# tub-rip/cmax_slam

Measured on AMD Instinct MI355X. Metric: warped-events/sec/GPU (1M ev, 640x480 IWE) + CMax iters/sec, higher is better.
Workload: dtype f64

## Files before the change

### cmax_slam_amd/csrc/cmx_binning.hip

```cpp
#include <mutex>
#include <cstring>

#include <rocprim/rocprim.hpp>

#include "cmx_internal.hpp"
#include "cmx_warp.hpp"
#include "cmx_fixed.hpp"
#include "cmx_tilepass.hpp"
#include "cmx_fusedgather.hpp"
#include "cmx_selfserve.hpp"

namespace cmx {

__device__ __forceinline__ uint32_t tile_key(int xx, int yy, bool ok, int W, int H, int tiles_x, uint32_t sentinel) {
  if (!ok) {
    if (xx < 1 - kBinMargin || xx >= W - 2 + kBinMargin || yy < 1 - kBinMargin || yy >= H - 2 + kBinMargin) return sentinel;
    xx = min(max(xx, 1), W - 3);
    yy = min(max(yy, 1), H - 3);
  }
  return (uint32_t)((yy / kBinTile) * tiles_x + xx / kBinTile);
}

__global__ __launch_bounds__(256) void fe_bin_keys_kernel(FeSplatArgs a, int tiles_x, int ntiles, uint32_t *keys,
                                                          uint32_t *idx) {
  fe_resolve_omega(a);
  for (int i = blockIdx.x * 256 + threadIdx.x; i < a.n; i += gridDim.x * 256) {
    const FeWarp w = fe_warp_event<false>(a, i);
    keys[i] = tile_key(w.xx, w.yy, w.ok, a.W, a.H, tiles_x, (uint32_t)ntiles);
    idx[i] = (uint32_t)i;
  }
}
__global__ __launch_bounds__(256) void be_bin_keys_kernel(BeSplatArgs a, int tiles_x, int ntiles, uint32_t *keys,
                                                          uint32_t *idx) {
  for (int i = blockIdx.x * 256 + threadIdx.x; i < a.n; i += gridDim.x * 256) {
    const BeWarp w = be_warp_event<0>(a, i);
    const uint32_t t = tile_key(w.xx, w.yy, w.ok, a.Wp, a.Hp, tiles_x, (uint32_t)ntiles);
    keys[i] = t == (uint32_t)ntiles ? (uint32_t)(2 * ntiles) : 2 * t + (w.is_old ? 0u : 1u);
    idx[i] = (uint32_t)i;
  }
}
static int grid_for(int n) {
  int b = (n + 255) / 256;
  return b < 1 ? 1 : (b > 2048 ? 2048 : b);
}
void launch_fe_bin_keys(const FeSplatArgs &a, int tiles_x, int ntiles, uint32_t *keys, uint32_t *idx, hipStream_t s) {
  hipLaunchKernelGGL(fe_bin_keys_kernel, dim3(grid_for(a.n)), dim3(256), 0, s, a, tiles_x, ntiles, keys, idx);
}
void launch_be_bin_keys(const BeSplatArgs &a, int tiles_x, int ntiles, uint32_t *keys, uint32_t *idx, hipStream_t s) {
  hipLaunchKernelGGL(be_bin_keys_kernel, dim3(grid_for(a.n)), dim3(256), 0, s, a, tiles_x, ntiles, keys, idx);
}

int sort_pairs_u32(void *temp, size_t *temp_bytes, const uint32_t *kin, uint32_t *kout, const uint32_t *vin,
                   uint32_t *vout, unsigned n, int end_bit, hipStream_t s) {
  return (int)rocprim::radix_sort_pairs(temp, *temp_bytes, kin, kout, vin, vout, n, 0, end_bit, s);
}

__global__ __launch_bounds__(256) void apply_perm_kernel(const uint32_t *xy, const uint32_t *idx_sorted, int per_batch,
                                                         int n, uint32_t *sxy, uint32_t *sbatch) {
  for (int j = blockIdx.x * 256 + threadIdx.x; j < n; j += gridDim.x * 256) {
    const uint32_t i = idx_sorted[j];
    sxy[j] = xy[i];
    sbatch[j] = i / (uint32_t)per_batch;
  }
}
void launch_apply_perm(const uint32_t *xy, const uint32_t *idx_sorted, int per_batch, int n, uint32_t *sxy,
                       uint32_t *sbatch, hipStream_t s) {
  hipLaunchKernelGGL(apply_perm_kernel, dim3(grid_for(n)), dim3(256), 0, s, xy, idx_sorted, per_batch, n, sxy, sbatch);
}

__global__ void tile_lower_bound_kernel(const uint32_t *keys, int n, int count, int *tile_start) {
  const int t = blockIdx.x * blockDim.x + threadIdx.x;
  if (t >= count) return;
  int lo = 0, hi = n;
  while (lo < hi) {
    const int mid = (lo + hi) >> 1;
    if (keys[mid] < (uint32_t)t) lo = mid + 1;
    else hi = mid;
  }
  tile_start[t] = lo;
}
void launch_tile_lower_bound(const uint32_t *keys_sorted, int n, int count, int *tile_start, hipStream_t s) {
  hipLaunchKernelGGL(tile_lower_bound_kernel, dim3((count + 255) / 256), dim3(256), 0, s, keys_sorted, n, count, tile_start);
}

constexpr int kCountSortMaxBins = 16400;
constexpr int kBinBlock = 1024;
constexpr int kBinMaxSlices = 512;
extern __shared__ int hist_sh[];

__device__ __forceinline__ void hist_zero(int nbins) {
  for (int k = threadIdx.x; k < nbins; k += kBinBlock) hist_sh[k] = 0;
  __syncthreads();
}
__device__ __forceinline__ void hist_store_row(int nbins, int *table) {
  __syncthreads();
  int *row = table + (size_t)blockIdx.x * nbins;
  for (int k = threadIdx.x; k < nbins; k += kBinBlock) row[k] = hist_sh[k];
}
__global__ __launch_bounds__(kBinBlock) void fe_bin_hist_kernel(FeSplatArgs a, int tiles_x, int ntiles, int per_block,
                                                                uint32_t *keys, int *table) {
  fe_resolve_omega(a);
  hist_zero(ntiles + 1);
  const int beg = blockIdx.x * per_block, end = min(a.n, beg + per_block);
  for (int i = beg + threadIdx.x; i < end; i += kBinBlock) {
    const FeWarp w = fe_warp_event<false>(a, i);
    const uint32_t key = tile_key(w.xx, w.yy, w.ok, a.W, a.H, tiles_x, (uint32_t)ntiles);
    keys[i] = key;
    atomicAdd(&hist_sh[key], 1);
  }
  hist_store_row(ntiles + 1, table);
}
__global__ __launch_bounds__(kBinBlock) void be_bin_hist_kernel(BeSplatArgs a, int tiles_x, int ntiles, int per_block,
                                                                uint32_t *keys, int *table) {
  hist_zero(2 * ntiles + 1);
  const int beg = blockIdx.x * per_block, end = min(a.n, beg + per_block);
  for (int i = beg + threadIdx.x; i < end; i += kBinBlock) {
    const BeWarp w = be_warp_event<0>(a, i);
    const uint32_t t = tile_key(w.xx, w.yy, w.ok, a.Wp, a.Hp, tiles_x, (uint32_t)ntiles);
    const uint32_t key = t == (uint32_t)ntiles ? (uint32_t)(2 * ntiles) : 2 * t + (w.is_old ? 0u : 1u);
    keys[i] = key;
    atomicAdd(&hist_sh[key], 1);
  }
  hist_store_row(2 * ntiles + 1, table);
}
__global__ __launch_bounds__(256) void column_scan_kernel(int *table, int nbins, int nslices, int *total) {
  const int k = blockIdx.x * 256 + threadIdx.x;
  if (k >= nbins) return;
  int run = 0, s = 0;
  for (; s + 8 <= nslices; s += 8) {
    int v[8];
#pragma unroll
    for (int q = 0; q < 8; q++) v[q] = table[(size_t)(s + q) * nbins + k];
#pragma unroll
    for (int q = 0; q < 8; q++) {
      table[(size_t)(s + q) * nbins + k] = run;
      run += v[q];
    }
  }
  for (; s < nslices; s++) {
    const int v = table[(size_t)s * nbins + k];
    table[(size_t)s * nbins + k] = run;
    run += v;
  }
  total[k] = run;
}
__global__ __launch_bounds__(kBinBlock) void scan_bins_kernel(const int *total, int nbins, int *tile_start) {
  __shared__ int wave_tot[kBinBlock / 64];
  const int tid = threadIdx.x, lane = tid & 63, wave = tid >> 6;
  const int per = (nbins + kBinBlock - 1) / kBinBlock;
  const int k0 = min(nbins, tid * per), k1 = min(nbins, k0 + per);
  int sum = 0;
  for (int k = k0; k < k1; k++) sum += total[k];
  int incl = sum;
#pragma unroll
  for (int o = 1; o < 64; o <<= 1) {
    const int v = __shfl_up(incl, o, 64);
    if (lane >= o) incl += v;
  }
// ... 160 lines not shown
    __shared__ int nact_sh;
    if (tid == 0) nact_sh = 0;
    int *nch = ts_sh;
    int mine[(kRankSortMax + 1023) / 1024];
#pragma unroll
    for (int q = 0; q < (kRankSortMax + 1023) / 1024; q++) {
      const int t = tid + q * 1024;
      int len = t < ntiles ? tile_start[t + 1] - tile_start[t] : 0;
      if (len < 0) len = 0;
      mine[q] = len / M + (len % M ? 1 : 0);
    }
    __syncthreads();
#pragma unroll
    for (int q = 0; q < (kRankSortMax + 1023) / 1024; q++)
      if (tid + q * 1024 < ntiles) nch[tid + q * 1024] = mine[q];
    __syncthreads();
    for (int t = tid; t < ntiles; t += 1024) {
      const int tx = t % tiles_x, ty = t / tiles_x;
      int sum = 0;
      for (int dy = -kFuseNbr; dy <= kFuseNbr; dy++)
        for (int dx = -kFuseNbr; dx <= kFuseNbr; dx++) {
          const int ux = tx + dx, uy = ty + dy;
          if (ux >= 0 && ux < tiles_x && uy >= 0 && uy < fused.tiles_y) sum += nch[uy * tiles_x + ux];
        }
      for (int h = 0; h < kFuseStrips; h++) {
        const int u = t * kFuseStrips + h;
        fused.nbr_expected[u] = sum;
        fused.nbr_cnt[(size_t)u * kFuseCntStride] = 0u;
        fused.partials[u] = 0.0;
        fused.partials[ntiles * kFuseStrips + u] = 0.0;
      }
      if (sum > 0) atomicAdd(&nact_sh, kFuseStrips);
    }
    __syncthreads();
    if (tid == 0) {
      if (fused.n_active) *fused.n_active = nact_sh;
      if (fused.tiles_done) *fused.tiles_done = 0u;
    }
  }
}
bool fused_tables_ok(int ntiles, int planes_per_tile) { return planes_per_tile == 1 && ntiles + 2 <= kRankSortMax + 2; }
void launch_build_chunks(const int *tile_start, int ntiles, int planes_per_tile, int tiles_x, int margin, int M, Chunk *chunks,
                         int *count, unsigned long long *count_host, unsigned binning_id, hipStream_t s, const FusedTables *fused) {
  FusedTables ft{};
  if (fused && fused_tables_ok(ntiles, planes_per_tile)) ft = *fused;
  hipLaunchKernelGGL(build_chunks_kernel, dim3(1), dim3(1024), 0, s, tile_start, ntiles, planes_per_tile, tiles_x, margin, M,
                     chunks, count, count_host, binning_id, ft);
}

__device__ __forceinline__ void lds_add_fix(fix_t *p, fix_t v) {
  __hip_atomic_fetch_add(p, v, __ATOMIC_RELAXED, __HIP_MEMORY_SCOPE_WORKGROUP);
}
__device__ __forceinline__ void vote4_lds(fix_t *win, int lx, int ly, float dx, float dy) {
  fix_t *q = win + ly * kBinStride + lx;
  lds_add_fix(q, to_fix((1.f - dx) * (1.f - dy)));
  lds_add_fix(q + 1, to_fix(dx * (1.f - dy)));
  lds_add_fix(q + kBinStride, to_fix((1.f - dx) * dy));
  lds_add_fix(q + kBinStride + 1, to_fix(dx * dy));
}

__global__ __launch_bounds__(256) void fixed_to_float_kernel(fix_t *fixed, float *planes, size_t n) {
  for (size_t i = (size_t)blockIdx.x * 256 + threadIdx.x; i < n; i += (size_t)gridDim.x * 256) {
    const fix_t v = fixed[i];
    if (v != 0ull) {
      planes[i] = (float)((double)v * kFixInv);
      fixed[i] = 0ull;
    }
  }
}
void launch_fixed_to_float(unsigned long long *fixed, float *planes, size_t n, hipStream_t s) {
  if (n == 0) return;
  size_t blocks = (n + 1023) / 1024;
  if (blocks > 4096) blocks = 4096;
  hipLaunchKernelGGL(fixed_to_float_kernel, dim3((unsigned)blocks), dim3(256), 0, s, fixed, planes, n);
}

static_assert(kBinWindow * kBinWindow % 256 == 0, "window cells per thread");
constexpr int kUnroll = 2;

#ifndef CMX_FE_SPLAT_NT
#define CMX_FE_SPLAT_NT 512
#endif
constexpr int kFeSplatNT = CMX_FE_SPLAT_NT;
static_assert(kBinWindow * kBinWindow % kFeSplatNT == 0, "window cells per thread");
static_assert(sizeof(fix_t) * kBinWindow * kBinStride >= kTpLdsBytes, "the fused tile pass reuses the vote window's LDS");
constexpr unsigned long long kFuseTimeoutTicks = 200000ull;
template <bool FIXED, bool STREAM, int FUSE>
__device__ __forceinline__ void fe_splat_lds_body(FeSplatArgs &a, const BinnedEvents &b, const FusedArgs &f) {
  __shared__ __attribute__((aligned(16))) fix_t win[kBinWindow * kBinStride];
  if (wg_stop_requested(a.skip)) return;
  if (FUSE == 2 && (int)blockIdx.x >= b.nchunks + f.tiles_x * f.tiles_y * kFuseStrips) {
    __shared__ FgSmem fg_sm;
    fused_gather_role<kFeSplatNT>(a, b, f, (int)blockIdx.x - b.nchunks - f.tiles_x * f.tiles_y * kFuseStrips, fg_sm);
    return;
  }
  if ((FUSE == 1 || FUSE == 2) && (int)blockIdx.x >= b.nchunks) {
    const int t = (int)blockIdx.x - b.nchunks;
    const unsigned expected = (unsigned)f.nbr_expected[t];
    if (f.trace && threadIdx.x == 0) { f.trace[8 * (size_t)blockIdx.x] = wall_clock64(); f.trace[8 * (size_t)blockIdx.x + 3] = expected ? 2 : 3; }
    if (expected == 0u || (f.debug & 1)) return;
    __shared__ int ok_sh;
    auto wait_inputs = [&]() -> bool {
      if (threadIdx.x == 0) {
        const unsigned long long t0 = wall_clock64();
        int ok = 1;
        while (__hip_atomic_load(f.nbr_cnt + (size_t)t * kFuseCntStride, __ATOMIC_RELAXED, __HIP_MEMORY_SCOPE_AGENT) < expected) {
          if (f.debug & 8) __builtin_amdgcn_s_sleep(32); else if (f.debug & 16) __builtin_amdgcn_s_sleep(127); else __builtin_amdgcn_s_sleep(2);
          if (wall_clock64() - t0 > kFuseTimeoutTicks) { ok = 0; break; }
        }
        if (ok) __hip_atomic_store(f.nbr_cnt + (size_t)t * kFuseCntStride, 0u, __ATOMIC_RELAXED, __HIP_MEMORY_SCOPE_AGENT);
        else atomicOr(b.fallback, kFuseIncomplete);
// ... 12 lines not shown
        __hip_atomic_store(f.tile_done + (size_t)t * kFuseCntStride, f.seq, __ATOMIC_RELAXED, __HIP_MEMORY_SCOPE_AGENT);
        __hip_atomic_fetch_add(f.tiles_done, 1u, __ATOMIC_RELAXED, __HIP_MEMORY_SCOPE_AGENT);
      }
    }
    if (f.trace && threadIdx.x == 0) { asm volatile("s_waitcnt vmcnt(0)" ::: "memory"); f.trace[8 * (size_t)blockIdx.x + 2] = wall_clock64(); }
    return;
  }
  fe_resolve_omega(a);
  Chunk c = b.chunks[blockIdx.x];
  if (FUSE && f.trace && threadIdx.x == 0) { f.trace[8 * (size_t)blockIdx.x] = wall_clock64(); f.trace[8 * (size_t)blockIdx.x + 3] = 0; }
  const bool has_chunk = (int)blockIdx.x < *b.nchunks_dev;
  if (!has_chunk) {
    if (FUSE != 3) return;
    c = Chunk{-200000000, -200000000, 0, 0, 0, -1};
  }
  const bool has_win = c.wx0 > -100000000;
  const int tid = threadIdx.x;
  __shared__ unsigned sfall;
  if (tid == 0) sfall = 0;
  if (has_win)
    for (int p = tid; p < kBinWindow * kBinStride; p += kFeSplatNT) win[p] = 0ull;
  __syncthreads();
  unsigned nfall = 0;
  for (int j0 = c.beg + tid; j0 < c.end; j0 += kFeSplatNT * kUnroll) {
    bool act[kUnroll];
    double px[kUnroll], py[kUnroll], pz[kUnroll], dt[kUnroll];
    if (STREAM) {
#pragma unroll
      for (int u = 0; u < kUnroll; u++) {
        const int j = j0 + u * kFeSplatNT;
        act[u] = j < c.end;
        const int jj = act[u] ? j : c.beg;
        const double2 v = *reinterpret_cast<const double2 *>(b.sb + 2 * (size_t)jj);
        px[u] = v.x; py[u] = v.y; pz[u] = 1.0;
        dt[u] = b.sdt[jj];
      }
    } else {
      uint32_t e[kUnroll], bi[kUnroll];
#pragma unroll
      for (int u = 0; u < kUnroll; u++) {
        const int j = j0 + u * kFeSplatNT;
        act[u] = j < c.end;
        e[u] = act[u] ? b.sxy[j] : 0u;
        bi[u] = act[u] ? b.sbatch[j] : 0u;
      }
#pragma unroll
      for (int u = 0; u < kUnroll; u++) {
        load_bearing(a, (int)(e[u] & 0xffff), (int)((e[u] >> 16) & 0x7fff), px[u], py[u], pz[u]);
        dt[u] = a.batch_dt[bi[u]];
      }
    }
#pragma unroll
    for (int u = 0; u < kUnroll; u++) {
      const FeWarp w = fe_warp_math<false>(a, px[u], py[u], pz[u], dt[u]);
      if (act[u] && w.ok) {
        const int lx = w.xx - c.wx0, ly = w.yy - c.wy0;
        if (has_win && lx >= 0 && lx < kBinWindow - 1 && ly >= 0 && ly < kBinWindow - 1) {
          vote4_lds(win, lx, ly, w.dx, w.dy);
        } else {
          if (FIXED) vote4_global_fix(b.fixed, a.W, w.xx, w.yy, w.dx, w.dy);
          else vote4_global(a.planes, a.W, w.xx, w.yy, w.dx, w.dy);
          nfall++;
          if (!has_win || lx < kBinMargin - kFuseReach || lx + 1 > kBinMargin + kBinTile - 1 + kFuseReach || ly < kBinMargin - kFuseReach ||
              ly + 1 > kBinMargin + kBinTile - 1 + kFuseReach)
            nfall |= kFuseUnsafe;
        }
      }
    }
  }
  if (nfall) {
    atomicAdd(&sfall, nfall & kFuseCountMask);
    if (nfall & kFuseUnsafe) atomicOr(&sfall, kFuseUnsafe);
  }
  __syncthreads();
  if (tid == 0 && sfall) {
    if (sfall & kFuseCountMask) atomicAdd(b.fallback, sfall & kFuseCountMask);
    if (sfall & kFuseUnsafe) atomicOr(b.fallback, kFuseUnsafe);
  }
  if (has_win) {
    constexpr int kCells = kBinWindow * kBinWindow / kFeSplatNT;
    fix_t cell[kCells];
#pragma unroll
    for (int k = 0; k < kCells; k++) {
      const int p = tid + kFeSplatNT * k, ly = p / kBinWindow, lx = p - ly * kBinWindow;
      cell[k] = win[ly * kBinStride + lx];
    }
#pragma unroll
    for (int k = 0; k < kCells; k++) {
      const fix_t v = cell[k];
      if (v != 0ull) {
        const int p = tid + kFeSplatNT * k, ly = p / kBinWindow, lx = p - ly * kBinWindow;
        const size_t at = (size_t)(c.wy0 + ly) * a.W + (c.wx0 + lx);
        if (FIXED) atomicAdd(b.fixed + at, v);
        else atomic_add_f32(a.planes + at, (float)((double)v * kFixInv));
      }
    }
  }
  if (FUSE) {
    asm volatile("s_waitcnt vmcnt(0)" ::: "memory");
    __syncthreads();
    constexpr int kSide = 2 * kFuseNbr + 1;
    if (c.tile >= 0 && tid < kSide * kSide * kFuseStrips && !(f.debug & 4)) {
      const int q = tid / kFuseStrips, h = tid % kFuseStrips;
      const int tx = c.tile % f.tiles_x + (q % kSide - kFuseNbr), ty = c.tile / f.tiles_x + (q / kSide - kFuseNbr);
      if (tx >= 0 && tx < f.tiles_x && ty >= 0 && ty < f.tiles_y)
        __hip_atomic_fetch_add(f.nbr_cnt + (size_t)((ty * f.tiles_x + tx) * kFuseStrips + h) * kFuseCntStride, 1u, __ATOMIC_RELAXED,
                               __HIP_MEMORY_SCOPE_AGENT);
    }
    if (f.trace && tid == 0) { f.trace[8 * (size_t)blockIdx.x + 1] = wall_clock64(); f.trace[8 * (size_t)blockIdx.x + 3] = 1; }
  }
// ... 60 lines not shown
  } else {
    if (stream) launch_fe_splat_lds_t<false, true, 0>(a, b, none, s, t0, t1);
    else launch_fe_splat_lds_t<false, false, 0>(a, b, none, s, t0, t1);
  }
}

template <bool FIXED>
__global__ __launch_bounds__(256) void be_splat_lds_kernel(BeSplatArgs a, BinnedEvents b) {
  __shared__ fix_t win[kBinWindow * kBinStride];
  const Chunk c = b.chunks[blockIdx.x];
  if ((int)blockIdx.x >= *b.nchunks_dev) return;
  const bool has_win = c.wx0 > -100000000;
  const int tid = threadIdx.x;
  const size_t np = (size_t)a.Wp * a.Hp;
  __shared__ unsigned sfall;
  if (tid == 0) sfall = 0;
  if (has_win)
    for (int p = tid; p < kBinWindow * kBinStride; p += 256) win[p] = 0ull;
  __syncthreads();
  unsigned nfall = 0;
  constexpr int U = 2;
  for (int j0 = c.beg + tid; j0 < c.end; j0 += 256 * U) {
    uint32_t e[U], bi[U];
    bool act[U];
#pragma unroll
    for (int u = 0; u < U; u++) {
      const int j = j0 + u * 256;
      act[u] = j < c.end;
      e[u] = act[u] ? b.sxy[j] : 0u;
      bi[u] = act[u] ? b.sbatch[j] : 0u;
    }
    double rx[U], ry[U], rz[U];
#pragma unroll
    for (int u = 0; u < U; u++) {
      double R[9];
      const double *Rp = a.poseR[bi[u]].R;
#pragma unroll
      for (int k = 0; k < 9; k++) R[k] = Rp[k];
      if (b.sb) {
        const int jj = act[u] ? j0 + u * 256 : c.beg;
        const double2 v = *reinterpret_cast<const double2 *>(b.sb + 2 * (size_t)jj);
        be_rotate<true>(R, v.x, v.y, 1.0, rx[u], ry[u], rz[u]);
      } else {
        double b0, b1, b2;
        load_bearing(a, (int)(e[u] & 0xffff), (int)((e[u] >> 16) & 0x7fff), b0, b1, b2);
        be_rotate<false>(R, b0, b1, b2, rx[u], ry[u], rz[u]);
      }
    }
#pragma unroll
    for (int u = 0; u < U; u++) {
      const BeWarp w = be_project<0>(a, e[u], (int)bi[u], rx[u], ry[u], rz[u]);
      if (act[u] && w.ok) {
        const int lx = w.xx - c.wx0, ly = w.yy - c.wy0;
        if (has_win && lx >= 0 && lx < kBinWindow - 1 && ly >= 0 && ly < kBinWindow - 1) {
          vote4_lds(win, lx, ly, w.dx, w.dy);
        } else {
          if (FIXED) vote4_global_fix(b.fixed + (w.is_old ? 0 : np), a.Wp, w.xx, w.yy, w.dx, w.dy);
          else vote4_global(a.planes + (w.is_old ? 0 : np), a.Wp, w.xx, w.yy, w.dx, w.dy);
          if (b.tflags) {
            b.tflags[(w.yy / kTileY) * b.tflags_tiles_x + w.xx / kTileX] = 1;
            b.tflags[(w.yy / kTileY) * b.tflags_tiles_x + (w.xx + 1) / kTileX] = 1;
            b.tflags[((w.yy + 1) / kTileY) * b.tflags_tiles_x + w.xx / kTileX] = 1;
            b.tflags[((w.yy + 1) / kTileY) * b.tflags_tiles_x + (w.xx + 1) / kTileX] = 1;
          }
          nfall++;
        }
      }
    }
  }
  if (nfall) atomicAdd(&sfall, nfall);
  __syncthreads();
  if (tid == 0 && sfall) atomicAdd(b.fallback, sfall);
  if (has_win) {
    const size_t plane_off = c.plane ? np : 0;
    constexpr int kCells = kBinWindow * kBinWindow / 256;
    fix_t cell[kCells];
#pragma unroll
    for (int k = 0; k < kCells; k++) {
      const int p = tid + 256 * k, ly = p / kBinWindow, lx = p - ly * kBinWindow;
      cell[k] = win[ly * kBinStride + lx];
    }
#pragma unroll
    for (int k = 0; k < kCells; k++) {
      const fix_t v = cell[k];
      if (v != 0ull) {
        const int p = tid + 256 * k, ly = p / kBinWindow, lx = p - ly * kBinWindow;
        const size_t at = plane_off + (size_t)(c.wy0 + ly) * a.Wp + (c.wx0 + lx);
        if (FIXED) atomicAdd(b.fixed + at, v);
        else atomic_add_f32(a.planes + at, (float)((double)v * kFixInv));
        if (b.tflags) b.tflags[((c.wy0 + ly) / kTileY) * b.tflags_tiles_x + (c.wx0 + lx) / kTileX] = 1;
      }
    }
  }
}
void launch_be_splat_lds(const BeSplatArgs &a, const BinnedEvents &b, hipStream_t s, hipEvent_t t0, hipEvent_t t1) {
  if (b.nchunks <= 0) return;
  if (b.fixed) {
    if (t0 || t1) hipExtLaunchKernelGGL(be_splat_lds_kernel<true>, dim3(b.nchunks), dim3(256), 0, s, t0, t1, 0, a, b);
    else hipLaunchKernelGGL(be_splat_lds_kernel<true>, dim3(b.nchunks), dim3(256), 0, s, a, b);
  } else {
    if (t0 || t1) hipExtLaunchKernelGGL(be_splat_lds_kernel<false>, dim3(b.nchunks), dim3(256), 0, s, t0, t1, 0, a, b);
    else hipLaunchKernelGGL(be_splat_lds_kernel<false>, dim3(b.nchunks), dim3(256), 0, s, a, b);
  }
}

}
```

### cmax_slam_amd/csrc/cmx_kernels.hip

```cpp
#include "../../include/cmax_hip.h"
#include "cmx_internal.hpp"
#include "cmx_warp.hpp"

#define CMX_LAUNCH(kernel, grid, block, lds, stream, t0, t1, ...)                                            \
  do {                                                                                                      \
    if ((t0) || (t1)) hipExtLaunchKernelGGL(kernel, grid, block, lds, stream, t0, t1, 0, __VA_ARGS__);      \
    else hipLaunchKernelGGL(kernel, grid, block, lds, stream, __VA_ARGS__);                                 \
  } while (0)
namespace cmx {

template <bool DERIV>
__global__ __launch_bounds__(256) void fe_splat_kernel(FeSplatArgs a) {
  const int W = a.W;
  const size_t np = (size_t)W * a.H;
  for (int i = blockIdx.x * 256 + threadIdx.x; i < a.n; i += gridDim.x * 256) {
    const FeWarp w = fe_warp_event<DERIV>(a, i);
    if (w.ok) {
      const float dx = w.dx, dy = w.dy;
      float *q = a.planes + (size_t)w.yy * W + w.xx;
      atomic_add_f32(q, (1.f - dx) * (1.f - dy));
      atomic_add_f32(q + 1, dx * (1.f - dy));
      atomic_add_f32(q + W, (1.f - dx) * dy);
      atomic_add_f32(q + W + 1, dx * dy);
      if (DERIV) {
// ... 1422 lines not shown
    else CMX_LAUNCH((image_adjoint_kernel<-1, kAdjTX, kAdjTY, kAdjThreads, true>), g, dim3(kAdjThreads), lds, s, t0, t1, a);
  } else {
    const dim3 g(a.img.nblk);
    if (a.img.r == 4) CMX_LAUNCH((image_adjoint_kernel<4, kAdjTX, kAdjTY, kAdjThreads, false>), g, dim3(kAdjThreads), lds, s, t0, t1, a);
    else CMX_LAUNCH((image_adjoint_kernel<-1, kAdjTX, kAdjTY, kAdjThreads, false>), g, dim3(kAdjThreads), lds, s, t0, t1, a);
  }
}

__device__ __forceinline__ void bilinear_grad(const float *it, int W, int xx, int yy, float dx, float dy, float &A, float &B) {
  const float *q = it + (size_t)yy * W + xx;
  const float i00 = q[0], i01 = q[1], i10 = q[W], i11 = q[W + 1];
  A = (1.f - dy) * (i01 - i00) + dy * (i11 - i10);
  B = (1.f - dx) * (i10 - i00) + dx * (i11 - i01);
}

__device__ __forceinline__ void border_grad(const float *cx, const float *cy, int W, int H, int r, int xx, int yy, float dx,
                                            float dy, float &A, float &B) {
  A = 0.f;
  B = 0.f;
  if (xx <= r || xx + 1 >= W - 1 - r || yy <= r || yy + 1 >= H - 1 - r) {
    const float c00 = cx[xx] * cy[yy], c01 = cx[xx + 1] * cy[yy], c10 = cx[xx] * cy[yy + 1], c11 = cx[xx + 1] * cy[yy + 1];
    A = (1.f - dy) * (c01 - c00) + dy * (c11 - c10);
    B = (1.f - dx) * (c10 - c00) + dx * (c11 - c01);
  }
}

int gather_blocks(int n) {
  int blocks = (n + 255) / 256;
  const int cap = 768;
  return blocks < 1 ? 1 : (blocks > cap ? cap : blocks);
}
#ifndef CMX_FE_GATHER_NT
#define CMX_FE_GATHER_NT 256
#endif
#ifndef CMX_FE_GATHER_PER_BLOCK
#define CMX_FE_GATHER_PER_BLOCK 1024
#endif
constexpr int kFeGatherNT = CMX_FE_GATHER_NT;
constexpr int kFeGatherPerBlock = CMX_FE_GATHER_PER_BLOCK, kFeGatherCap = 2048;
int fe_gather_blocks(int n) {
  int per = kFeGatherPerBlock;
  if (n < 512 * 1024) {
    per = ((n / 512 + kFeGatherNT - 1) / kFeGatherNT) * kFeGatherNT;
    per = per < kFeGatherNT ? kFeGatherNT : (per > kFeGatherPerBlock ? kFeGatherPerBlock : per);
  }
  int blocks = (n + per - 1) / per;
  return blocks < 1 ? 1 : (blocks > kFeGatherCap ? kFeGatherCap : blocks);
}

template <int U>
__device__ __forceinline__ void fe_gather_streams(const FeGatherArgs &g, const FeSplatArgs &a, int blk_beg, int blk_end, double acc[3],
                                                  double acc2[3]) {
  const int W = a.W, H = a.H, r = g.r;
  for (int i0 = blk_beg + (int)threadIdx.x; i0 < blk_end; i0 += kFeGatherNT * U) {
    double2 bv[U];
    double dt[U];
    bool ok[U];
#pragma unroll
    for (int u = 0; u < U; u++) {
      const int i = i0 + u * kFeGatherNT;
      ok[u] = i < blk_end;
      const int ii = ok[u] ? i : blk_beg;
      bv[u] = *reinterpret_cast<const double2 *>(g.sb + 2 * (size_t)ii);
      dt[u] = g.sdt[ii];
    }
    FeWarp w[U];
    const float *q[U];
#pragma unroll
    for (int u = 0; u < U; u++) {
      w[u] = fe_warp_math<true>(a, bv[u].x, bv[u].y, 1.0, dt[u]);
      ok[u] = ok[u] && w[u].ok;
      q[u] = g.itilde + (ok[u] ? (size_t)w[u].yy * W + w[u].xx : (size_t)0);
    }
    float i00[U], i01[U], i10[U], i11[U];
#pragma unroll
    for (int u = 0; u < U; u++) { i00[u] = q[u][0]; i01[u] = q[u][1]; i10[u] = q[u][W]; i11[u] = q[u][W + 1]; }
    bool edge = false;
#pragma unroll
    for (int u = 0; u < U; u++) {
      const float dx = w[u].dx, dy = w[u].dy;
      const float A = (1.f - dy) * (i01[u] - i00[u]) + dy * (i11[u] - i10[u]);
      const float B = (1.f - dx) * (i10[u] - i00[u]) + dx * (i11[u] - i01[u]);
#pragma unroll
      for (int k = 0; k < 3; k++) {
        const double t = (double)w[u].r0[k] * (double)A + (double)w[u].r1[k] * (double)B;
        acc[k] = ok[u] ? acc[k] + t : acc[k];
      }
      edge = edge || (ok[u] && (w[u].xx <= r || w[u].xx + 1 >= W - 1 - r || w[u].yy <= r || w[u].yy + 1 >= H - 1 - r));
    }
    if (g.cx && __any(edge)) {
#pragma unroll
      for (int u = 0; u < U; u++) {
        if (!ok[u]) continue;
        float Ac, Bc;
        border_grad(g.cx, g.cy, W, H, r, w[u].xx, w[u].yy, w[u].dx, w[u].dy, Ac, Bc);
        if (Ac != 0.f || Bc != 0.f) {
#pragma unroll
          for (int k = 0; k < 3; k++) acc2[k] += (double)w[u].r0[k] * (double)Ac + (double)w[u].r1[k] * (double)Bc;
        }
      }
    }
  }
}
#ifndef CMX_FE_GATHER_U
#define CMX_FE_GATHER_U 4
#endif

template <int CHAIN>
__global__ __launch_bounds__(kFeGatherNT) void fe_gather_kernel(FeGatherArgs g) {
  if (CHAIN != 2 && g.gate && *g.gate == 0) return;
  if (CHAIN && wg_stop_requested(g.ev.skip)) return;
  __shared__ double red[(kFeGatherNT / 64) * 6];
  __shared__ FinSmem fin_sm;
  if (CHAIN == 2) {
    const FinalizeArgs &fa = g.tail.fin;
    double s0, s1, mu;
    chain_moment_sums(fa.macc, s0, s1);
    const double c = contrast_from_sums(s0, s1, fa.npix, fa.measure, &mu);
    if (!fa.chain.sm_src && !gate_condition(c, fa.chain.gate_cur->thr, fa.chain.gate_cur->mode)) {
      if (blockIdx.x != 0) return;
      FinalizeArgs f = fa;
      f.gP = 0;
      f.gacc = nullptr;
      finalize_body<kFeGatherNT, true>(f, fin_sm);
      return;
    }
  }
  if (CHAIN) fe_resolve_omega(g.ev);
  const FeSplatArgs &a = g.ev;
  double acc[3] = {0, 0, 0}, acc2[3] = {0, 0, 0};
  constexpr int U = 2;
  const int per_block = ((a.n + (int)gridDim.x - 1) / (int)gridDim.x + kFeGatherNT - 1) / kFeGatherNT * kFeGatherNT;
  const int blk_beg = blockIdx.x * per_block, blk_end = min(a.n, blk_beg + per_block);
  const int stride = kFeGatherNT;
  if (CHAIN == 0 && CMX_FE_GATHER_U > 0 && g.sb) fe_gather_streams<(CMX_FE_GATHER_U > 0 ? CMX_FE_GATHER_U : 1)>(g, a, blk_beg, blk_end, acc, acc2);
  else
  for (int i0 = blk_beg + threadIdx.x; i0 < blk_end; i0 += stride * U) {
    double dt[U], px[U], py[U], pz[U];
    bool act[U];
    if (g.sb) {
#pragma unroll
      for (int u = 0; u < U; u++) {
        const int i = i0 + u * stride;
        act[u] = i < blk_end;
        const int ii = act[u] ? i : blk_beg;
        const double2 v = *reinterpret_cast<const double2 *>(g.sb + 2 * (size_t)ii);
        px[u] = v.x; py[u] = v.y; pz[u] = 1.0;
        dt[u] = g.sdt[ii];
      }
    } else {
      if (g.tb && !g.sxy) {
#pragma unroll
        for (int u = 0; u < U; u++) {
          const int i = i0 + u * stride;
          act[u] = i < blk_end;
          const int ii = act[u] ? i : blk_beg;
          const double2 v = *reinterpret_cast<const double2 *>(g.tb + 2 * (size_t)ii);
          px[u] = v.x; py[u] = v.y; pz[u] = 1.0;
          dt[u] = a.batch_dt[ii / a.per_batch];
        }
      } else {
      uint32_t e[U];
#pragma unroll
      for (int u = 0; u < U; u++) {
        const int i = i0 + u * stride;
        act[u] = i < blk_end;
        if (g.sxy) {
          e[u] = act[u] ? g.sxy[i] : 0u;
          dt[u] = act[u] ? a.batch_dt[g.sbatch[i]] : 0.0;
        } else {
          e[u] = act[u] ? a.xy[i] : 0u;
          dt[u] = act[u] ? a.batch_dt[i / a.per_batch] : 0.0;
        }
      }
#pragma unroll
      for (int u = 0; u < U; u++) {
        load_bearing(a, (int)(e[u] & 0xffff), (int)((e[u] >> 16) & 0x7fff), px[u], py[u], pz[u]);
      }
      }
    }
#pragma unroll
    for (int u = 0; u < U; u++) {
      const FeWarp w = fe_warp_math<true>(a, px[u], py[u], pz[u], dt[u]);
      if (act[u] && w.ok) {
        float A, B;
        bilinear_grad(g.itilde, a.W, w.xx, w.yy, w.dx, w.dy, A, B);
#pragma unroll
        for (int k = 0; k < 3; k++) acc[k] += (double)w.r0[k] * (double)A + (double)w.r1[k] * (double)B;
        if (g.cx) {
          float Ac, Bc;
          border_grad(g.cx, g.cy, a.W, a.H, g.r, w.xx, w.yy, w.dx, w.dy, Ac, Bc);
          if (Ac != 0.f || Bc != 0.f) {
#pragma unroll
            for (int k = 0; k < 3; k++) acc2[k] += (double)w.r0[k] * (double)Ac + (double)w.r1[k] * (double)Bc;
          }
        }
      }
    }
  }
  double v[6];
#pragma unroll
  for (int k = 0; k < 3; k++) v[k] = wave_sum(acc[k]);
  const bool any2 = g.cx && __any(acc2[0] != 0.0 || acc2[1] != 0.0 || acc2[2] != 0.0);
#pragma unroll
  for (int k = 0; k < 3; k++) v[3 + k] = any2 ? wave_sum(acc2[k]) : 0.0;
  const int wave = threadIdx.x >> 6, lane = threadIdx.x & 63;
  if (lane == 0) {
#pragma unroll
    for (int k = 0; k < 6; k++) red[wave * 6 + k] = v[k];
  }
  __syncthreads();
  const bool tail = g.tail.counters != nullptr;
  if (threadIdx.x < (g.cx ? 6 : 3)) {
    const int k = threadIdx.x;
    double v = red[k] + red[6 + k] + red[12 + k] + red[18 + k];
#pragma unroll
    for (int wv = 4; wv < kFeGatherNT / 64; wv++) v += red[6 * wv + k];
    if (g.tail.fin.gacc) {
      if (v != 0.0)
        __hip_atomic_fetch_add(g.tail.fin.gacc + (size_t)(blockIdx.x % kTailShards) * g.tail.fin.gacc_stride + k, v, __ATOMIC_RELAXED,
                               __HIP_MEMORY_SCOPE_AGENT);
    } else if (tail) st_sc1(g.gpartials + (size_t)k * gridDim.x + blockIdx.x, v);
    else g.gpartials[(size_t)k * gridDim.x + blockIdx.x] = v;
  }
  if (CHAIN == 0 && tail && g.tail.poll) {
    asm volatile("s_waitcnt vmcnt(0)" ::: "memory");
    __syncthreads();
    constexpr int kLines = kTailShards + 1;
    if (blockIdx.x != 0) {
      if (threadIdx.x == 0)
        __hip_atomic_fetch_add(g.tail.counters + (blockIdx.x % kLines) * kTailStride, 1u, __ATOMIC_RELAXED, __HIP_MEMORY_SCOPE_AGENT);
      return;
    }
    if (threadIdx.x < 64) {
      const unsigned want = gridDim.x - 1u;
      const unsigned long long t0 = wall_clock64();
      const int q = threadIdx.x;
      for (;;) {
        unsigned v = q < kLines ? __hip_atomic_load(g.tail.counters + q * kTailStride, __ATOMIC_RELAXED, __HIP_MEMORY_SCOPE_AGENT) : 0u;
#pragma unroll
        for (int o = 8; o >= 1; o >>= 1) v += __shfl_xor(v, o, 64);
        const unsigned total = __shfl(v, 0, 64);
        if (total >= want) break;
        __builtin_amdgcn_s_sleep(1);
        if (wall_clock64() - t0 > 100000000ull) {
          if (q == 0 && g.tail.fin.fallback) atomicOr(g.tail.fin.fallback, kFuseIncomplete);
          break;
        }
// ... 688 lines not shown
```

### cmax_slam_amd/csrc/cmx_warp.hpp

```cpp
#pragma once
#include "cmx_internal.hpp"
#include "cmx_trig.hpp"

namespace cmx {

__device__ __forceinline__ void atomic_add_f32(float *p, float v) {
  __hip_atomic_fetch_add(p, v, __ATOMIC_RELAXED, __HIP_MEMORY_SCOPE_AGENT);
}

template <typename Args>
__device__ __forceinline__ void load_bearing(const Args &a, int ex, int ey, double &b0, double &b1, double &b2) {
  const size_t i = (size_t)ey * a.W + ex;
  if (a.lut2) {
    const double2 v = *reinterpret_cast<const double2 *>(a.lut2 + 2 * i);
    b0 = v.x; b1 = v.y; b2 = 1.0;
  } else {
    const double *l = a.lut + 3 * i;
    b0 = l[0]; b1 = l[1]; b2 = l[2];
  }
}

__device__ __forceinline__ void fe_resolve_omega(FeSplatArgs &a) {
  if (a.w_dev) { a.wx = a.w_dev[0]; a.wy = a.w_dev[1]; a.wz = a.w_dev[2]; }
}

__device__ __forceinline__ bool wg_stop_requested(const int *skip) {
  if (!skip) return false;
  __shared__ int stop_sh;
  if (threadIdx.x == 0) stop_sh = __hip_atomic_load(skip, __ATOMIC_RELAXED, __HIP_MEMORY_SCOPE_SYSTEM);
  __syncthreads();
  return stop_sh != 0;
}

struct FeWarp {
  int xx, yy;
  float dx, dy;
  bool ok;
  float r0[3], r1[3];
};

template <bool DERIV>
__device__ __forceinline__ FeWarp fe_warp_math(const FeSplatArgs &a, double px, double py, double pz, double dt) {
  FeWarp w;
  const double drx = a.wx * dt, dry = a.wy * dt, drz = a.wz * dt;
  const double rx = px + (dry * pz - drz * py);
  const double ry = py + (drz * px - drx * pz);
  const double rz = pz + (drx * py - dry * px);
  const double iz = 1.0 / rz;
  const double cxn = rx * iz, cyn = ry * iz;
  const double u = a.fx * cxn + a.cx;
  const double v = a.fy * cyn + a.cy;
  w.xx = (int)u;
  w.yy = (int)v;
  w.ok = (1 <= w.xx && w.xx < a.W - 2 && 1 <= w.yy && w.yy < a.H - 2);
  w.dx = (float)(u - w.xx);
  w.dy = (float)(v - w.yy);
  if (DERIV) {
    const double vx = (-dt) * px, vy = (-dt) * py, vz = (-dt) * pz;
    const double a02 = -cxn * iz, a12 = -cyn * iz;
    w.r0[0] = (float)(a.fx * (a02 * (-vy)));
    w.r0[1] = (float)(a.fx * (iz * (-vz) + a02 * vx));
    w.r0[2] = (float)(a.fx * (iz * vy));
    w.r1[0] = (float)(a.fy * (iz * vz + a12 * (-vy)));
    w.r1[1] = (float)(a.fy * (a12 * vx));
    w.r1[2] = (float)(a.fy * (iz * (-vx)));
  }
  return w;
}

template <bool DERIV>
__device__ __forceinline__ FeWarp fe_warp_core(const FeSplatArgs &a, uint32_t e, double dt) {
  const int ex = e & 0xffff, ey = (e >> 16) & 0x7fff;
  double b0, b1, b2;
  load_bearing(a, ex, ey, b0, b1, b2);
  return fe_warp_math<DERIV>(a, b0, b1, b2, dt);
}

template <bool DERIV>
__device__ __forceinline__ FeWarp fe_warp_event(const FeSplatArgs &a, int i) {
  return fe_warp_core<DERIV>(a, a.xy[i], a.batch_dt[i / a.per_batch]);
}

struct BeWarp {
  int xx, yy;
  float dx, dy;
  bool ok, is_old;
  int batch;
  float m[6];
};

template <bool Z1>
__device__ __forceinline__ void be_rotate(const double *R, double b0, double b1, double b2, double &x, double &y, double &z) {
  if (Z1) {
    x = __builtin_fma(R[0], b0, __builtin_fma(R[1], b1, R[2]));
    y = __builtin_fma(R[3], b0, __builtin_fma(R[4], b1, R[5]));
    z = __builtin_fma(R[6], b0, __builtin_fma(R[7], b1, R[8]));
  } else {
    x = __builtin_fma(R[0], b0, __builtin_fma(R[1], b1, R[2] * b2));
    y = __builtin_fma(R[3], b0, __builtin_fma(R[4], b1, R[5] * b2));
    z = __builtin_fma(R[6], b0, __builtin_fma(R[7], b1, R[8] * b2));
  }
}

template <int DERIV>
__device__ __forceinline__ BeWarp be_project(const BeSplatArgs &a, uint32_t e, int batch, double x, double y, double z) {
  BeWarp w;
  w.is_old = (e >> 31) != 0;
  w.batch = batch;
  double pxm, pym, rho;
  {
#pragma clang fp contract(fast)
    const double phi = lean_atan2(x, z);
    const double rho2 = x * x + (y * y + z * z);
    double inv_rho = __builtin_amdgcn_rsq(rho2);
    const double h = 0.5 * rho2;
    inv_rho = inv_rho * (1.5 - (h * inv_rho) * inv_rho);
    inv_rho = inv_rho * (1.5 - (h * inv_rho) * inv_rho);
    rho = rho2 * inv_rho;
    const double theta = lean_asin(y * inv_rho);
    pxm = a.cxp + phi * a.fx;
    pym = a.cyp + theta * a.fy;
  }
  w.xx = (int)pxm;
  w.yy = (int)pym;
  w.ok = (1 <= w.xx && w.xx < a.Wp - 2 && 1 <= w.yy && w.yy < a.Hp - 2);
  w.dx = (float)(pxm - w.xx);
  w.dy = (float)(pym - w.yy);
  if (DERIV == 2) {
    const float xf = (float)x, yf = (float)y, zf = (float)z, rhof = (float)rho;
    const float fxf = (float)a.fx, fyf = (float)a.fy;
    const float inv_rho = __builtin_amdgcn_rcpf(rhof), inv_z = __builtin_amdgcn_rcpf(zf);
// ... 58 lines not shown
```

Baseline: 28.56 billion.

## Refactor FE gradient into fused double-precision term and vectorize LDS vote

Replaces the per-event float Jacobian rows with a new DERIV=2 path that keeps iz/cxn/cyn and computes the gradient contribution directly in double via FMA chains. It also swaps 1/rz for an rcp-plus-Newton reciprocal, uses unsigned single-compare range checks, vectorizes the bilinear LDS vote weights with packed float2 FMA, and adds a waves_per_eu hint to the gather kernel. The edge path now recomputes the warp using g.sdt, which costs extra work but only when events are near the border. The aim is fewer instructions and registers in the hot splat and gather loops, with a small change in rounding behavior.

```diff
diff --git a/cmax_slam_amd/csrc/cmx_binning.hip b/cmax_slam_amd/csrc/cmx_binning.hip
--- a/cmax_slam_amd/csrc/cmx_binning.hip
+++ b/cmax_slam_amd/csrc/cmx_binning.hip
@@ -25,7 +25,7 @@
                                                           uint32_t *idx) {
   fe_resolve_omega(a);
   for (int i = blockIdx.x * 256 + threadIdx.x; i < a.n; i += gridDim.x * 256) {
-    const FeWarp w = fe_warp_event<false>(a, i);
+    const FeWarp w = fe_warp_event<0>(a, i);
     keys[i] = tile_key(w.xx, w.yy, w.ok, a.W, a.H, tiles_x, (uint32_t)ntiles);
     idx[i] = (uint32_t)i;
   }
@@ -103,7 +103,7 @@
   hist_zero(ntiles + 1);
   const int beg = blockIdx.x * per_block, end = min(a.n, beg + per_block);
   for (int i = beg + threadIdx.x; i < end; i += kBinBlock) {
-    const FeWarp w = fe_warp_event<false>(a, i);
+    const FeWarp w = fe_warp_event<0>(a, i);
     const uint32_t key = tile_key(w.xx, w.yy, w.ok, a.W, a.H, tiles_x, (uint32_t)ntiles);
     keys[i] = key;
     atomicAdd(&hist_sh[key], 1);
@@ -370,11 +370,16 @@
   __hip_atomic_fetch_add(p, v, __ATOMIC_RELAXED, __HIP_MEMORY_SCOPE_WORKGROUP);
 }
 __device__ __forceinline__ void vote4_lds(fix_t *win, int lx, int ly, float dx, float dy) {
+  typedef float f32x2 __attribute__((ext_vector_type(2)));
   fix_t *q = win + ly * kBinStride + lx;
-  lds_add_fix(q, to_fix((1.f - dx) * (1.f - dy)));
-  lds_add_fix(q + 1, to_fix(dx * (1.f - dy)));
-  lds_add_fix(q + kBinStride, to_fix((1.f - dx) * dy));
-  lds_add_fix(q + kBinStride + 1, to_fix(dx * dy));
+  const f32x2 wx = {1.f - dx, dx};
+  const f32x2 top = wx * (f32x2){1.f - dy, 1.f - dy}, bot = wx * (f32x2){dy, dy};
+  const f32x2 ft = __builtin_elementwise_fma(top, (f32x2){kFixScale, kFixScale}, (f32x2){0.5f, 0.5f});
+  const f32x2 fb = __builtin_elementwise_fma(bot, (f32x2){kFixScale, kFixScale}, (f32x2){0.5f, 0.5f});
+  lds_add_fix(q, (fix_t)(unsigned)ft.x);
+  lds_add_fix(q + 1, (fix_t)(unsigned)ft.y);
+  lds_add_fix(q + kBinStride, (fix_t)(unsigned)fb.x);
+  lds_add_fix(q + kBinStride + 1, (fix_t)(unsigned)fb.y);
 }
 
 __global__ __launch_bounds__(256) void fixed_to_float_kernel(fix_t *fixed, float *planes, size_t n) {
@@ -493,10 +498,10 @@
     }
 #pragma unroll
     for (int u = 0; u < kUnroll; u++) {
-      const FeWarp w = fe_warp_math<false>(a, px[u], py[u], pz[u], dt[u]);
+      const FeWarp w = fe_warp_math<0>(a, px[u], py[u], pz[u], dt[u]);
       if (act[u] && w.ok) {
         const int lx = w.xx - c.wx0, ly = w.yy - c.wy0;
-        if (has_win && lx >= 0 && lx < kBinWindow - 1 && ly >= 0 && ly < kBinWindow - 1) {
+        if (has_win && in_range(lx, 0, kBinWindow - 1) && in_range(ly, 0, kBinWindow - 1)) {
           vote4_lds(win, lx, ly, w.dx, w.dy);
         } else {
           if (FIXED) vote4_global_fix(b.fixed, a.W, w.xx, w.yy, w.dx, w.dy);
@@ -663,7 +668,7 @@
       const BeWarp w = be_project<0>(a, e[u], (int)bi[u], rx[u], ry[u], rz[u]);
       if (act[u] && w.ok) {
         const int lx = w.xx - c.wx0, ly = w.yy - c.wy0;
-        if (has_win && lx >= 0 && lx < kBinWindow - 1 && ly >= 0 && ly < kBinWindow - 1) {
+        if (has_win && in_range(lx, 0, kBinWindow - 1) && in_range(ly, 0, kBinWindow - 1)) {
           vote4_lds(win, lx, ly, w.dx, w.dy);
         } else {
           if (FIXED) vote4_global_fix(b.fixed + (w.is_old ? 0 : np), a.Wp, w.xx, w.yy, w.dx, w.dy);
diff --git a/cmax_slam_amd/csrc/cmx_kernels.hip b/cmax_slam_amd/csrc/cmx_kernels.hip
--- a/cmax_slam_amd/csrc/cmx_kernels.hip
+++ b/cmax_slam_amd/csrc/cmx_kernels.hip
@@ -1498,6 +1498,7 @@
 __device__ __forceinline__ void fe_gather_streams(const FeGatherArgs &g, const FeSplatArgs &a, int blk_beg, int blk_end, double acc[3],
                                                   double acc2[3]) {
   const int W = a.W, H = a.H, r = g.r;
+  const int in_x = max(W - 3 - 2 * r, 0), in_y = max(H - 3 - 2 * r, 0);
   for (int i0 = blk_beg + (int)threadIdx.x; i0 < blk_end; i0 += kFeGatherNT * U) {
     double2 bv[U];
     double dt[U];
@@ -1512,38 +1513,34 @@
     }
     FeWarp w[U];
     const float *q[U];
+    bool edge = false;
 #pragma unroll
     for (int u = 0; u < U; u++) {
-      w[u] = fe_warp_math<true>(a, bv[u].x, bv[u].y, 1.0, dt[u]);
+      w[u] = fe_warp_math<2>(a, bv[u].x, bv[u].y, 1.0, dt[u]);
+      dt[u] *= w[u].iz;
       ok[u] = ok[u] && w[u].ok;
-      q[u] = g.itilde + (ok[u] ? (size_t)w[u].yy * W + w[u].xx : (size_t)0);
+      q[u] = g.itilde + (ok[u] ? (size_t)(unsigned)w[u].yy * (unsigned)W + (unsigned)w[u].xx : (size_t)0);
+      edge = edge || (ok[u] && !(in_range(w[u].xx, r + 1, in_x) && in_range(w[u].yy, r + 1, in_y)));
     }
     float i00[U], i01[U], i10[U], i11[U];
 #pragma unroll
     for (int u = 0; u < U; u++) { i00[u] = q[u][0]; i01[u] = q[u][1]; i10[u] = q[u][W]; i11[u] = q[u][W + 1]; }
-    bool edge = false;
 #pragma unroll
     for (int u = 0; u < U; u++) {
       const float dx = w[u].dx, dy = w[u].dy;
-      const float A = (1.f - dy) * (i01[u] - i00[u]) + dy * (i11[u] - i10[u]);
-      const float B = (1.f - dx) * (i10[u] - i00[u]) + dx * (i11[u] - i01[u]);
-#pragma unroll
-      for (int k = 0; k < 3; k++) {
-        const double t = (double)w[u].r0[k] * (double)A + (double)w[u].r1[k] * (double)B;
-        acc[k] = ok[u] ? acc[k] + t : acc[k];
-      }
-      edge = edge || (ok[u] && (w[u].xx <= r || w[u].xx + 1 >= W - 1 - r || w[u].yy <= r || w[u].yy + 1 >= H - 1 - r));
+      float A = ok[u] ? (1.f - dy) * (i01[u] - i00[u]) + dy * (i11[u] - i10[u]) : 0.f;
+      float B = ok[u] ? (1.f - dx) * (i10[u] - i00[u]) + dx * (i11[u] - i01[u]) : 0.f;
+      asm("" : "+v"(A), "+v"(B));
+      fe_grad_term(a, w[u], bv[u].x, bv[u].y, 1.0, dt[u], A, B, acc);
     }
     if (g.cx && __any(edge)) {
 #pragma unroll
       for (int u = 0; u < U; u++) {
         if (!ok[u]) continue;
+        const FeWarp wb = fe_warp_math<2>(a, bv[u].x, bv[u].y, 1.0, g.sdt[i0 + u * kFeGatherNT]);
         float Ac, Bc;
-        border_grad(g.cx, g.cy, W, H, r, w[u].xx, w[u].yy, w[u].dx, w[u].dy, Ac, Bc);
-        if (Ac != 0.f || Bc != 0.f) {
-#pragma unroll
-          for (int k = 0; k < 3; k++) acc2[k] += (double)w[u].r0[k] * (double)Ac + (double)w[u].r1[k] * (double)Bc;
-        }
+        border_grad(g.cx, g.cy, W, H, r, wb.xx, wb.yy, wb.dx, wb.dy, Ac, Bc);
+        if (Ac != 0.f || Bc != 0.f) fe_grad_term(a, wb, bv[u].x, bv[u].y, 1.0, dt[u], Ac, Bc, acc2);
       }
     }
   }
@@ -1553,7 +1550,7 @@
 #endif
 
 template <int CHAIN>
-__global__ __launch_bounds__(kFeGatherNT) void fe_gather_kernel(FeGatherArgs g) {
+__global__ __launch_bounds__(kFeGatherNT) __attribute__((amdgpu_waves_per_eu(4, 8))) void fe_gather_kernel(FeGatherArgs g) {
   if (CHAIN != 2 && g.gate && *g.gate == 0) return;
   if (CHAIN && wg_stop_requested(g.ev.skip)) return;
   __shared__ double red[(kFeGatherNT / 64) * 6];
@@ -1627,19 +1624,16 @@
     }
 #pragma unroll
     for (int u = 0; u < U; u++) {
-      const FeWarp w = fe_warp_math<true>(a, px[u], py[u], pz[u], dt[u]);
+      const FeWarp w = fe_warp_math<2>(a, px[u], py[u], pz[u], dt[u]);
       if (act[u] && w.ok) {
         float A, B;
         bilinear_grad(g.itilde, a.W, w.xx, w.yy, w.dx, w.dy, A, B);
-#pragma unroll
-        for (int k = 0; k < 3; k++) acc[k] += (double)w.r0[k] * (double)A + (double)w.r1[k] * (double)B;
+        const double k = dt[u] * w.iz;
+      fe_grad_term(a, w, px[u], py[u], pz[u], k, A, B, acc);
         if (g.cx) {
           float Ac, Bc;
           border_grad(g.cx, g.cy, a.W, a.H, g.r, w.xx, w.yy, w.dx, w.dy, Ac, Bc);
-          if (Ac != 0.f || Bc != 0.f) {
-#pragma unroll
-            for (int k = 0; k < 3; k++) acc2[k] += (double)w.r0[k] * (double)Ac + (double)w.r1[k] * (double)Bc;
-          }
+          if (Ac != 0.f || Bc != 0.f) fe_grad_term(a, w, px[u], py[u], pz[u], k, Ac, Bc, acc2);
         }
       }
     }
diff --git a/cmax_slam_amd/csrc/cmx_warp.hpp b/cmax_slam_amd/csrc/cmx_warp.hpp
--- a/cmax_slam_amd/csrc/cmx_warp.hpp
+++ b/cmax_slam_amd/csrc/cmx_warp.hpp
@@ -37,25 +37,40 @@
   float dx, dy;
   bool ok;
   float r0[3], r1[3];
+  double iz, cxn, cyn;
 };
 
-template <bool DERIV>
+__device__ __forceinline__ double fe_recip(double d) {
+  double y = __builtin_amdgcn_rcp(d);
+  y = __builtin_fma(__builtin_fma(-d, y, 1.0), y, y);
+  y = __builtin_fma(__builtin_fma(-d, y, 1.0), y, y);
+  return __builtin_fma(__builtin_fma(-d, y, 1.0), y, y);
+}
+
+__device__ __forceinline__ bool in_range(int x, int lo, int n) { return (unsigned)x - (unsigned)lo < (unsigned)n; }
+
+template <int DERIV>
 __device__ __forceinline__ FeWarp fe_warp_math(const FeSplatArgs &a, double px, double py, double pz, double dt) {
   FeWarp w;
   const double drx = a.wx * dt, dry = a.wy * dt, drz = a.wz * dt;
   const double rx = px + (dry * pz - drz * py);
   const double ry = py + (drz * px - drx * pz);
   const double rz = pz + (drx * py - dry * px);
-  const double iz = 1.0 / rz;
+  const double iz = fe_recip(rz);
   const double cxn = rx * iz, cyn = ry * iz;
   const double u = a.fx * cxn + a.cx;
   const double v = a.fy * cyn + a.cy;
   w.xx = (int)u;
   w.yy = (int)v;
-  w.ok = (1 <= w.xx && w.xx < a.W - 2 && 1 <= w.yy && w.yy < a.H - 2);
+  w.ok = in_range(w.xx, 1, max(a.W - 3, 0)) && in_range(w.yy, 1, max(a.H - 3, 0));
   w.dx = (float)(u - w.xx);
   w.dy = (float)(v - w.yy);
-  if (DERIV) {
+  if (DERIV == 2) {
+    w.iz = iz;
+    w.cxn = cxn;
+    w.cyn = cyn;
+  }
+  if (DERIV == 1) {
     const double vx = (-dt) * px, vy = (-dt) * py, vz = (-dt) * pz;
     const double a02 = -cxn * iz, a12 = -cyn * iz;
     w.r0[0] = (float)(a.fx * (a02 * (-vy)));
@@ -68,7 +83,7 @@
   return w;
 }
 
-template <bool DERIV>
+template <int DERIV>
 __device__ __forceinline__ FeWarp fe_warp_core(const FeSplatArgs &a, uint32_t e, double dt) {
   const int ex = e & 0xffff, ey = (e >> 16) & 0x7fff;
   double b0, b1, b2;
@@ -76,7 +91,16 @@
   return fe_warp_math<DERIV>(a, b0, b1, b2, dt);
 }
 
-template <bool DERIV>
+__device__ __forceinline__ void fe_grad_term(const FeSplatArgs &a, const FeWarp &w, double px, double py, double pz, double k, float A,
+                                             float B, double acc[3]) {
+  const double gA = a.fx * (double)A, gB = a.fy * (double)B;
+  const double s = __builtin_fma(gB, w.cyn, gA * w.cxn);
+  acc[0] = __builtin_fma(k, __builtin_fma(-py, s, -(pz * gB)), acc[0]);
+  acc[1] = __builtin_fma(k, __builtin_fma(px, s, pz * gA), acc[1]);
+  acc[2] = __builtin_fma(k, __builtin_fma(px, gB, -(py * gA)), acc[2]);
+}
+
+template <int DERIV>
 __device__ __forceinline__ FeWarp fe_warp_event(const FeSplatArgs &a, int i) {
   return fe_warp_core<DERIV>(a, a.xy[i], a.batch_dt[i / a.per_batch]);
 }
```

Measured after the change: 28.57 billion (median of 2 runs). Within noise of the previous version (+0.0%).
